# zhyever/PatchFusion

Measured on NVIDIA H100. Metric: tiles/s, higher is better.
Workload: dtype bf16

## Files before the change

patchfusion_b200/csrc/pf_attn.cu:

```cuda
#include <stdlib.h>

#include "pf_common.cuh"
#include "pf_kernels.h"

namespace pf {

constexpr int kQTile = 128, kKTile = 128, kHd = 64;
constexpr int kAttnWG = 2;
constexpr int kAttnThreads = kAttnWG * 128 + 32;
constexpr int kKVStages = 3;
constexpr int kTileBytes = 16384;
constexpr int kOffQ = 0;
constexpr int kOffKV = kTileBytes;
constexpr int kOffBar = kOffKV + kKVStages * 2 * kTileBytes;
constexpr int kAttnSmem = 1024 + kOffBar + 256;

struct AttnParams {
  CUtensorMap tmQK;
  CUtensorMap tmVt;
  int B, seq, heads, D;
  int n_qt;
  float scale_log2;
  __nv_bfloat16* out;
  int out_ld;
};

__device__ __forceinline__ float ex2_approx(float x) {
  float y;
  asm("ex2.approx.ftz.f32 %0, %1;" : "=f"(y) : "f"(x));
  return y;
}

__global__ void __launch_bounds__(kAttnThreads, 1) pf_attention_kernel(const __grid_constant__ AttnParams P) {
  extern __shared__ uint8_t smem_raw[];
  uint8_t* smem = reinterpret_cast<uint8_t*>((reinterpret_cast<uintptr_t>(smem_raw) + 1023) & ~uintptr_t(1023));
  uint64_t* bars = reinterpret_cast<uint64_t*>(smem + kOffBar);
  uint64_t* q_full = bars;
  uint64_t* kv_full = bars + 1;
  uint64_t* kv_empty = kv_full + kKVStages;
  const int warp = threadIdx.x >> 5, lane = threadIdx.x & 31;
  const int qt = blockIdx.x % P.n_qt;
  const int bh = blockIdx.x / P.n_qt;
  const int b = bh / P.heads, head = bh - b * P.heads;
  const int n_kv = (P.seq + kKTile - 1) / kKTile;
  constexpr int kProducer = kAttnWG * 4;

  if (warp == kProducer && lane == 0) {
    prefetch_tmap(&P.tmQK);
    prefetch_tmap(&P.tmVt);
    mbar_init(q_full, 1);
    for (int s = 0; s < kKVStages; ++s) { mbar_init(&kv_full[s], 1); mbar_init(&kv_empty[s], kAttnWG * 4); }
    fence_barrier_init();
  }
  __syncthreads();
  pdl_launch_dependents();
  pdl_wait();

  if (warp == kProducer) {
    if (elect_one()) {
      mbar_expect_tx(q_full, kTileBytes);
      tma_load_3d(smem + kOffQ, &P.tmQK, q_full, head * kHd, qt * kQTile, b);
      int st = 0; uint32_t ph = 0;
      for (int j = 0; j < n_kv; ++j) {
        mbar_wait(&kv_empty[st], ph ^ 1);
        uint8_t* sk = smem + kOffKV + st * 2 * kTileBytes;
        mbar_expect_tx(&kv_full[st], 2 * kTileBytes);
        tma_load_3d(sk, &P.tmQK, &kv_full[st], P.D + head * kHd, j * kKTile, b);
        const int vrow = (b * P.heads + head) * kHd;
        tma_load_2d(sk + kTileBytes, &P.tmVt, &kv_full[st], j * kKTile, vrow);
        tma_load_2d(sk + kTileBytes + 8192, &P.tmVt, &kv_full[st], j * kKTile + 64, vrow);
        if (++st == kKVStages) { st = 0; ph ^= 1; }
      }
    }
    return;
  }

  const int g = warp >> 2, wq = warp & 3;
  mbar_wait(q_full, 0);
  uint32_t qf[4][4];
  {
    const uint32_t base = smem_u32(smem + kOffQ);
    const int row = 64 * g + 16 * wq + (lane & 15);
#pragma unroll
    for (int k = 0; k < 4; ++k)
      ldmatrix_x4(base + row * 128 + ((((2 * k) + (lane >> 4)) ^ (row & 7)) << 4), qf[k]);
  }
  float o[32];
#pragma unroll
  for (int i = 0; i < 32; ++i) o[i] = 0.f;
  float m0 = -INFINITY, m1 = -INFINITY, l0 = 0.f, l1 = 0.f;
  const float sl2 = P.scale_log2;
  int st = 0; uint32_t ph = 0;
  for (int j = 0; j < n_kv; ++j) {
    mbar_wait(&kv_full[st], ph);
    const uint32_t sk = smem_u32(smem + kOffKV + st * 2 * kTileBytes);
    float s[64];
    wgmma_fence();
#pragma unroll
    for (int k = 0; k < 4; ++k) Wgmma<128>::rs(s, qf[k], wgmma_desc_k128(sk) + 2 * k, k);
    wgmma_commit();
    wgmma_wait<0>();
    const int kv_left = P.seq - j * kKTile;
    if (kv_left < kKTile) {
#pragma unroll
      for (int i = 0; i < 64; ++i) {
        const int key = 8 * (i >> 2) + 2 * (lane & 3) + (i & 1);
        if (key >= kv_left) s[i] = -INFINITY;
      }
    }
    float x0 = -INFINITY, x1 = -INFINITY;
#pragma unroll
    for (int i = 0; i < 64; i += 4) {
      x0 = fmaxf(x0, fmaxf(s[i], s[i + 1]));
      x1 = fmaxf(x1, fmaxf(s[i + 2], s[i + 3]));
    }
#pragma unroll
    for (int d = 1; d < 4; d <<= 1) {
      x0 = fmaxf(x0, __shfl_xor_sync(0xffffffffu, x0, d));
      x1 = fmaxf(x1, __shfl_xor_sync(0xffffffffu, x1, d));
    }
    const float n0 = fmaxf(m0, x0 * sl2), n1 = fmaxf(m1, x1 * sl2);
    const float c0 = ex2_approx(m0 - n0), c1 = ex2_approx(m1 - n1);
    m0 = n0; m1 = n1;
    float r0 = 0.f, r1 = 0.f;
#pragma unroll
    for (int i = 0; i < 64; i += 4) {
      s[i] = ex2_approx(fmaf(s[i], sl2, -n0));
      s[i + 1] = ex2_approx(fmaf(s[i + 1], sl2, -n0));
      s[i + 2] = ex2_approx(fmaf(s[i + 2], sl2, -n1));
      s[i + 3] = ex2_approx(fmaf(s[i + 3], sl2, -n1));
      r0 += s[i] + s[i + 1];
      r1 += s[i + 2] + s[i + 3];
    }
    l0 = l0 * c0 + r0;
    l1 = l1 * c1 + r1;
#pragma unroll
    for (int i = 0; i < 32; i += 4) {
      o[i] *= c0; o[i + 1] *= c0;
      o[i + 2] *= c1; o[i + 3] *= c1;
    }
    wgmma_fence();
#pragma unroll
    for (int kk = 0; kk < 8; ++kk) {
      const uint32_t pa[4] = {pack_bf16(s[8 * kk], s[8 * kk + 1]), pack_bf16(s[8 * kk + 2], s[8 * kk + 3]),
                              pack_bf16(s[8 * kk + 4], s[8 * kk + 5]), pack_bf16(s[8 * kk + 6], s[8 * kk + 7])};
      Wgmma<64>::rs(o, pa, wgmma_desc_k128(sk + kTileBytes + (kk >> 2) * 8192) + 2 * (kk & 3), 1);
    }
    wgmma_commit();
    wgmma_wait<0>();
    __syncwarp();
    if (lane == 0) mbar_arrive(&kv_empty[st]);
    if (++st == kKVStages) { st = 0; ph ^= 1; }
  }
#pragma unroll
  for (int d = 1; d < 4; d <<= 1) {
    l0 += __shfl_xor_sync(0xffffffffu, l0, d);
    l1 += __shfl_xor_sync(0xffffffffu, l1, d);
  }
  const float i0 = 1.f / l0, i1 = 1.f / l1;
  const int q0 = qt * kQTile + 64 * g + 16 * wq + (lane >> 2);
  __nv_bfloat16* ob = P.out + static_cast<size_t>(b) * P.seq * P.out_ld + head * kHd + 2 * (lane & 3);
#pragma unroll
  for (int jd = 0; jd < 8; ++jd) {
    if (q0 < P.seq)
      *reinterpret_cast<uint32_t*>(ob + static_cast<size_t>(q0) * P.out_ld + 8 * jd) = pack_bf16(o[4 * jd] * i0, o[4 * jd + 1] * i0);
    if (q0 + 8 < P.seq)
      *reinterpret_cast<uint32_t*>(ob + static_cast<size_t>(q0 + 8) * P.out_ld + 8 * jd) =
          pack_bf16(o[4 * jd + 2] * i1, o[4 * jd + 3] * i1);
  }
}

}

using namespace pf;

extern "C" int pf_attention(const void* qk, int32_t qk_ld, const void* vt, int32_t B, int32_t seq, int32_t seq_pad,
                            int32_t heads, float scale, void* out, int32_t out_ld, void* stream) {
  static bool attr_done[kMaxDevices] = {false};
  const int dev = current_device();
  if (!attr_done[dev]) {
    cudaError_t e = cudaFuncSetAttribute(pf_attention_kernel, cudaFuncAttributeMaxDynamicSharedMemorySize, kAttnSmem);
    if (e != cudaSuccess) return set_error("cudaFuncSetAttribute(pf_attention_kernel): %s", cudaGetErrorString(e));
    attr_done[dev] = true;
  }
  const int D = heads * kHd;
  if (B < 1 || seq < 1 || heads < 1) return set_error("pf_attention: empty problem");
  if (qk_ld % 8 || seq_pad % 8 || out_ld % 8) return set_error("pf_attention: strides must be multiples of 8");
  if (seq_pad < seq) return set_error("pf_attention: seq_pad %d < seq %d", seq_pad, seq);
  AttnParams P;
  if (tmap_3d_bf16(&P.tmQK, qk, 2 * D, seq, B, qk_ld, static_cast<uint64_t>(seq) * qk_ld, 64, 128, 1)) return 1;
  if (tmap_2d_bf16(&P.tmVt, vt, seq, static_cast<uint64_t>(B) * heads * kHd, seq_pad, 64, 64)) return 1;
  P.B = B; P.seq = seq; P.heads = heads; P.D = D;
  P.n_qt = (seq + kQTile - 1) / kQTile;
  P.scale_log2 = scale * 1.4426950408889634f;
  P.out = static_cast<__nv_bfloat16*>(out);
  P.out_ld = out_ld;
  note_work(4.0 * B * heads * static_cast<double>(seq) * seq * kHd, "attention B%d heads%d seq%d", B, heads, seq);
  cudaError_t le = launch_pdl(pf_attention_kernel, dim3(B * heads * P.n_qt), dim3(kAttnThreads), kAttnSmem,
                              static_cast<cudaStream_t>(stream), P);
  if (le != cudaSuccess) return set_error("pf_attention_kernel launch: %s", cudaGetErrorString(le));
  return check_launch("pf_attention_kernel");
}
```

patchfusion_b200/csrc/pf_common.cuh:

```cuda
#pragma once
#include <cuda.h>
#include <cuda_bf16.h>
#include <cuda_runtime.h>
#include <stdint.h>

namespace pf {

__device__ __forceinline__ uint32_t smem_u32(const void* p) {
  return static_cast<uint32_t>(__cvta_generic_to_shared(p));
}

__device__ __forceinline__ uint32_t lane_id() { return threadIdx.x & 31; }

__device__ __forceinline__ bool elect_one() {
  uint32_t pred = 0;
  asm volatile(
      "{\n\t"
      ".reg .pred P1;\n\t"
      "elect.sync _|P1, 0xffffffff;\n\t"
      "selp.b32 %0, 1, 0, P1;\n\t"
      "}\n"
      : "=r"(pred));
  return pred != 0;
}

__device__ __forceinline__ void mbar_init(uint64_t* bar, uint32_t count) {
  asm volatile("mbarrier.init.shared::cta.b64 [%0], %1;" ::"r"(smem_u32(bar)), "r"(count) : "memory");
}
__device__ __forceinline__ void fence_barrier_init() {
  asm volatile("fence.mbarrier_init.release.cluster;" ::: "memory");
}
__device__ __forceinline__ void mbar_expect_tx(uint64_t* bar, uint32_t bytes) {
  asm volatile("mbarrier.arrive.expect_tx.shared::cta.b64 _, [%0], %1;" ::"r"(smem_u32(bar)), "r"(bytes) : "memory");
}
__device__ __forceinline__ void mbar_arrive(uint64_t* bar) {
  asm volatile("mbarrier.arrive.shared::cta.b64 _, [%0];" ::"r"(smem_u32(bar)) : "memory");
}
__device__ __forceinline__ bool mbar_try_wait(uint64_t* bar, uint32_t parity) {
  uint32_t ok;
  asm volatile(
      "{\n\t"
      ".reg .pred P1;\n\t"
      "mbarrier.try_wait.parity.shared::cta.b64 P1, [%1], %2, %3;\n\t"
      "selp.b32 %0, 1, 0, P1;\n\t"
      "}\n"
      : "=r"(ok)
      : "r"(smem_u32(bar)), "r"(parity), "r"(20000u)
      : "memory");
  return ok != 0;
}
__device__ __forceinline__ bool mbar_test_wait(uint64_t* bar, uint32_t parity) {
  uint32_t ok;
  asm volatile(
      "{\n\t"
      ".reg .pred P1;\n\t"
      "mbarrier.test_wait.parity.shared::cta.b64 P1, [%1], %2;\n\t"
      "selp.b32 %0, 1, 0, P1;\n\t"
      "}\n"
      : "=r"(ok)
      : "r"(smem_u32(bar)), "r"(parity)
      : "memory");
  return ok != 0;
}
__device__ __forceinline__ void mbar_wait(uint64_t* bar, uint32_t parity) {
  uint32_t spins = 0;
  while (!mbar_try_wait(bar, parity)) {
    if (++spins > (1u << 20)) { __trap(); }
  }
}

__device__ __forceinline__ void pdl_launch_dependents() { asm volatile("griddepcontrol.launch_dependents;" ::: "memory"); }
__device__ __forceinline__ void pdl_wait() { asm volatile("griddepcontrol.wait;" ::: "memory"); }

__device__ __forceinline__ void fence_proxy_async_smem() { asm volatile("fence.proxy.async.shared::cta;" ::: "memory"); }

__device__ __forceinline__ void prefetch_tmap(const CUtensorMap* m) {
  asm volatile("prefetch.tensormap [%0];" ::"l"(reinterpret_cast<uint64_t>(m)) : "memory");
}
__device__ __forceinline__ void tma_load_2d(void* dst, const CUtensorMap* m, uint64_t* bar, int c0, int c1) {
  asm volatile(
      "cp.async.bulk.tensor.2d.shared::cluster.global.mbarrier::complete_tx::bytes [%0], [%1, {%3, %4}], [%2];"
      ::"r"(smem_u32(dst)), "l"(reinterpret_cast<uint64_t>(m)), "r"(smem_u32(bar)), "r"(c0), "r"(c1)
      : "memory");
}
__device__ __forceinline__ void tma_load_2d_mc(void* dst, const CUtensorMap* m, uint64_t* bar, int c0, int c1, uint16_t mask) {
  asm volatile(
      "cp.async.bulk.tensor.2d.shared::cluster.global.mbarrier::complete_tx::bytes.multicast::cluster [%0], [%1, {%3, %4}], [%2], %5;"
      ::"r"(smem_u32(dst)), "l"(reinterpret_cast<uint64_t>(m)), "r"(smem_u32(bar)), "r"(c0), "r"(c1), "h"(mask)
      : "memory");
}
__device__ __forceinline__ uint32_t cluster_ctarank() {
  uint32_t r;
  asm volatile("mov.u32 %0, %%cluster_ctarank;" : "=r"(r));
  return r;
}
__device__ __forceinline__ void cluster_sync_all() {
  asm volatile("barrier.cluster.arrive.release.aligned;\n\tbarrier.cluster.wait.acquire.aligned;" ::: "memory");
}
__device__ __forceinline__ void tma_load_3d(void* dst, const CUtensorMap* m, uint64_t* bar, int c0, int c1, int c2) {
  asm volatile(
      "cp.async.bulk.tensor.3d.shared::cluster.global.mbarrier::complete_tx::bytes [%0], [%1, {%3, %4, %5}], [%2];"
      ::"r"(smem_u32(dst)), "l"(reinterpret_cast<uint64_t>(m)), "r"(smem_u32(bar)), "r"(c0), "r"(c1), "r"(c2)
      : "memory");
}
__device__ __forceinline__ void tma_load_4d(void* dst, const CUtensorMap* m, uint64_t* bar, int c0, int c1, int c2,
                                            int c3) {
  asm volatile(
      "cp.async.bulk.tensor.4d.shared::cluster.global.mbarrier::complete_tx::bytes [%0], [%1, {%3, %4, %5, %6}], [%2];"
      ::"r"(smem_u32(dst)), "l"(reinterpret_cast<uint64_t>(m)), "r"(smem_u32(bar)), "r"(c0), "r"(c1), "r"(c2),
      "r"(c3)
      : "memory");
}

__device__ __forceinline__ void tma_store_2d(const CUtensorMap* m, const void* src, int c0, int c1) {
  asm volatile("cp.async.bulk.tensor.2d.global.shared::cta.bulk_group [%0, {%2, %3}], [%1];"
               ::"l"(reinterpret_cast<uint64_t>(m)), "r"(smem_u32(src)), "r"(c0), "r"(c1) : "memory");
}
__device__ __forceinline__ void tma_store_4d(const CUtensorMap* m, const void* src, int c0, int c1, int c2, int c3) {
  asm volatile("cp.async.bulk.tensor.4d.global.shared::cta.bulk_group [%0, {%2, %3, %4, %5}], [%1];"
               ::"l"(reinterpret_cast<uint64_t>(m)), "r"(smem_u32(src)), "r"(c0), "r"(c1), "r"(c2), "r"(c3) : "memory");
}
__device__ __forceinline__ void tma_reduce_add_2d(const CUtensorMap* m, const void* src, int c0, int c1) {
  asm volatile("cp.reduce.async.bulk.tensor.2d.global.shared::cta.add.tile.bulk_group [%0, {%2, %3}], [%1];"
               ::"l"(reinterpret_cast<uint64_t>(m)), "r"(smem_u32(src)), "r"(c0), "r"(c1) : "memory");
}
__device__ __forceinline__ void bulk_commit() { asm volatile("cp.async.bulk.commit_group;" ::: "memory"); }
__device__ __forceinline__ void bulk_wait_read0() { asm volatile("cp.async.bulk.wait_group.read 0;" ::: "memory"); }
__device__ __forceinline__ void bulk_wait_read1() { asm volatile("cp.async.bulk.wait_group.read 1;" ::: "memory"); }
__device__ __forceinline__ void bulk_wait0() { asm volatile("cp.async.bulk.wait_group 0;" ::: "memory"); }
__device__ __forceinline__ void st_shared_v2f(uint32_t addr, float a, float b) {
  asm volatile("st.shared.v2.f32 [%0], {%1, %2};" ::"r"(addr), "f"(a), "f"(b) : "memory");
}
__device__ __forceinline__ void st_shared_v4(uint32_t addr, uint32_t a, uint32_t b, uint32_t c, uint32_t d) {
  asm volatile("st.shared.v4.b32 [%0], {%1, %2, %3, %4};" ::"r"(addr), "r"(a), "r"(b), "r"(c), "r"(d) : "memory");
}
__device__ __forceinline__ void ld_shared_v4(uint32_t addr, uint32_t& a, uint32_t& b, uint32_t& c, uint32_t& d) {
  asm volatile("ld.shared.v4.b32 {%0, %1, %2, %3}, [%4];" : "=r"(a), "=r"(b), "=r"(c), "=r"(d) : "r"(addr) : "memory");
}
__device__ __forceinline__ void mbar_arrive_cluster(uint64_t* bar, uint32_t cta) {
  uint32_t remote;
  asm volatile("mapa.shared::cluster.u32 %0, %1, %2;" : "=r"(remote) : "r"(smem_u32(bar)), "r"(cta));
  asm volatile("mbarrier.arrive.shared::cluster.b64 _, [%0];" ::"r"(remote) : "memory");
}

__device__ __forceinline__ void ldmatrix_x4(uint32_t addr, uint32_t (&r)[4]) {
  asm volatile("ldmatrix.sync.aligned.m8n8.x4.shared.b16 {%0, %1, %2, %3}, [%4];"
               : "=r"(r[0]), "=r"(r[1]), "=r"(r[2]), "=r"(r[3]) : "r"(addr) : "memory");
}

__device__ __forceinline__ void stmatrix_x4(uint32_t addr, uint32_t r0, uint32_t r1, uint32_t r2, uint32_t r3) {
  asm volatile("stmatrix.sync.aligned.m8n8.x4.shared.b16 [%0], {%1, %2, %3, %4};"
               ::"r"(addr), "r"(r0), "r"(r1), "r"(r2), "r"(r3) : "memory");
}

__device__ __forceinline__ uint64_t wgmma_desc_k128(uint32_t saddr) {
// ... 247 lines not shown
```

patchfusion_b200/csrc/pf_gemm.cu:

```cuda
#include "pf_common.cuh"
#include "pf_kernels.h"

namespace pf {

constexpr int kBlockM = 128;
constexpr int kBlockK = 64;
constexpr int kATileBytes = kBlockM * kBlockK * 2;
constexpr int kEpiWarps = 8;
constexpr int kGemmThreads = (kEpiWarps + 1) * 32;
constexpr int kHaloThreads = (kEpiWarps + 3) * 32;
constexpr int kRsWarp0 = kEpiWarps;
constexpr int kMaxSmem = 227 * 1024;
constexpr int kXposeWarp = 16 * 32 * 4;
constexpr int kStageWarp = 2 * kXposeWarp;
constexpr int kBarBytes = 512;

__host__ __device__ constexpr int gemm_stage_bytes(int bn) { return kATileBytes + bn * kBlockK * 2; }
__host__ __device__ constexpr int gemm_stages(int bn) {
  return (kMaxSmem - 1024  - kBarBytes - kEpiWarps * kStageWarp) / gemm_stage_bytes(bn) < 8
             ? (kMaxSmem - 1024 - kBarBytes - kEpiWarps * kStageWarp) / gemm_stage_bytes(bn)
             : 8;
}

struct GemmKernelParams {
// ... 725 lines not shown
            int dy = d.taps == 9 ? tap / 3 - 1 : 0;
            int dx = d.taps == 9 ? tap % 3 - 1 : 0;
            for (int ch = 0; ch < d.chunks[s]; ++ch, ++kb) {
              const long long tl_w = tl.now();
              mbar_wait(&empty_bar[stage], phase ^ 1);
              tl.add(1, tl_w);
              uint8_t* sa = smem + stage * stage_bytes;
              uint8_t* sb = sa + kATileBytes;
              if (elect_one()) {
                mbar_expect_tx(&full_bar[stage], stage_bytes);
                if (d.a_mode == 0) tma_load_2d(sa, &P.tmA[s], &full_bar[stage], ch * kBlockK, c.m0);
                else tma_load_4d(sa, &P.tmA[s], &full_bar[stage], ch * kBlockK, c.x0 + dx, c.y0 + dy, c.img);
                if (MC) {
                  constexpr int half_rows = BN / 2;
                  tma_load_2d_mc(sb + it.rank * half_rows * 128, &P.tmBh, &full_bar[stage], kb * kBlockK,
                                 c.n0 + it.rank * half_rows, static_cast<uint16_t>(3));
                } else {
                  tma_load_2d(sb, &P.tmB, &full_bar[stage], kb * kBlockK, c.n0);
                }
              }
              if (++stage == stages) { stage = 0; phase ^= 1; }
            }
          }
        }
      }
      tl.add(2, tl_start);
      if (lane == 0) tl.flush(0, 3);
    }
  } else {
    EpiTma et;
    et.tm = &P.tmOut; et.stg_ptr = xpose + warp * kStageWarp; et.stg = smem_u32(et.stg_ptr); et.cur = 0;
    float* buf = reinterpret_cast<float*>(et.stg_ptr);
    const uint32_t a_off = static_cast<uint32_t>((warp >> 2) * 64 * 128);
    float acc[BN / 2];
    int stage = 0; uint32_t phase = 0;
    int rs = 0;
    GemmTimeline tl;
    const long long tl_start = tl.now();
    for (int ti = it.first; ti < it.count; ti += it.step) {
      const TileCoord c = decode_tile(d, it.tile(ti));
      tl.tile();
      const long long tl_main = tl.now();
      uint32_t accum = 0;
      for (int kb = 0; kb < P.k_steps; ++kb) {
        const long long tl_w = tl.now();
        mbar_wait(&full_bar[stage], phase);
        tl.add(1, tl_w);
        const uint32_t sa = smem_u32(smem + stage * stage_bytes);
        const uint64_t adesc = wgmma_desc_k128(sa + a_off);
        const uint64_t bdesc = wgmma_desc_k128(sa + kATileBytes);
        wgmma_fence();
#pragma unroll
        for (int k = 0; k < kBlockK / 16; ++k) Wgmma<BN>::ss(acc, adesc + 2 * k, bdesc + 2 * k, accum | k);
        wgmma_commit();
        accum = 1;
        wgmma_wait<1>();
        if (kb > 0) {
          release_stage<CL>(&empty_bar[rs], lane);
          if (++rs == stages) rs = 0;
        }
        if (++stage == stages) { stage = 0; phase ^= 1; }
      }
      wgmma_wait<0>();
      release_stage<CL>(&empty_bar[rs], lane);
      if (++rs == stages) rs = 0;
      tl.add(2, tl_main);
      const long long tl_epi = tl.now();
      epilogue_tile(d, c, acc, warp, lane, buf, &et);
      __syncwarp();
      tl.add(3, tl_epi);
    }
    if (lane == 0) bulk_wait0();
    tl.add(4, tl_start);
    if (lane == 0 && (warp & 3) == 0) tl.flush(3, 5);
  }
  __syncthreads();
  if (MC) cluster_sync_all();
}

constexpr int kPpStageBytes = kATileBytes + kPpBN * kBlockK * 2;
constexpr int kPpStages = (kMaxSmem - 1024  - kBarBytes - kEpiWarps * kStageWarp) / kPpStageBytes;
static_assert(kPpStages == 6, "pf_gemm_pp_kernel operand ring");
constexpr int kPpTurnBar = 1;

template <int ID>
__device__ __forceinline__ void named_bar_sync256() { asm volatile("bar.sync %0, 256;" ::"n"(ID) : "memory"); }
template <int ID>
__device__ __forceinline__ void named_bar_arrive256() { asm volatile("bar.arrive %0, 256;" ::"n"(ID) : "memory"); }

template <int S, int SC = 0>
__device__ __forceinline__ void epilogue_tile_vt(const GemmDesc& d, const float (&acc)[S], const TileCoord& c, int warp,
                                                 int lane) {
  const int q = lane & 3;
  int ro[2];
#pragma unroll
  for (int h = 0; h < 2; ++h) {
    const int m = c.m0 + 16 * warp + (lane >> 2) + 8 * h;
    const int b = m / d.vt_seq, tok = m - b * d.vt_seq;
    ro[h] = m < d.M ? b * d.vt_dim * d.vt_seq_pad + tok : -1;
  }
  for (int ch = 0; 32 * ch < 2 * S; ++ch) {
    const int lcol = c.n0 + ch * 32;
    if (lcol >= d.n_logical) break;
    float v[16];
    acc_chunk(ch, acc, v);
    if constexpr (SC != 0) epi_dequant(d, v, lcol + 2 * q, d.a_scale);
    epi_frag(d, v, lcol + 2 * q, false);
#pragma unroll
    for (int j = 0; j < 4; ++j) {
#pragma unroll
      for (int e = 0; e < 2; ++e) {
        const int n = lcol + 8 * j + 2 * q + e;
        if (n >= d.n_logical) continue;
        __nv_bfloat16* vp = d.vt + (n - d.vt_col0) * d.vt_seq_pad;
        if (ro[0] >= 0) vp[ro[0]] = __float2bfloat16(v[4 * j + e]);
        if (ro[1] >= 0) vp[ro[1]] = __float2bfloat16(v[4 * j + 2 + e]);
      }
    }
  }
}

template <bool F8, int S>
__device__ __forceinline__ void epilogue_tile_pp(const GemmDesc& d, EpiTma& et, const float (&acc)[S], const TileCoord& c,
                                                 int warp, int lane) {
  constexpr int SC = F8 ? 2 : 0;
  if (d.vt != nullptr && c.n0 >= d.vt_col0) epilogue_tile_vt<S, SC>(d, acc, c, warp, lane);
  else if (d.tma_out == 2) epilogue_tile_tma_f32<S, SC>(d, et, acc, c, warp, lane);
  else {
    if constexpr (F8) {
      if (d.out_e4m3) {
        epilogue_tile_tma_e4m3<S, true>(d, et, acc, c, warp, lane);
        return;
      }
    }
    epilogue_tile_tma_bf16<64, S, SC>(d, et, acc, c, warp, lane);
  }
}

template <bool MC, bool F8>
__device__ __forceinline__ void gemm_pp_body(const GemmKernelParams& P) {
  constexpr int CL = MC ? 2 : 1;
  constexpr int kKBlock = F8 ? 2 * kBlockK : kBlockK;
  extern __shared__ uint8_t smem_raw[];
  const GemmDesc& d = P.d;
  uint8_t* smem = reinterpret_cast<uint8_t*>((reinterpret_cast<uintptr_t>(smem_raw) + 1023) & ~uintptr_t(1023));
  uint8_t* stg = smem + kPpStages * kPpStageBytes;
  uint64_t* full_bar = reinterpret_cast<uint64_t*>(stg + kEpiWarps * kStageWarp);
  uint64_t* empty_bar = full_bar + kPpStages;

  const int warp = __shfl_sync(0xffffffffu, static_cast<int>(threadIdx.x >> 5), 0);
  const int lane = threadIdx.x & 31;
  pdl_launch_dependents();

  constexpr int kTmaWarp = kEpiWarps;
  if (warp == kTmaWarp && lane == 0) {
    prefetch_tmap(&P.tmA[0]);
    prefetch_tmap(MC ? &P.tmBh : &P.tmB);
    for (int s = 0; s < kPpStages; ++s) { mbar_init(&full_bar[s], 1); mbar_init(&empty_bar[s], 4 * CL); }
    prefetch_tmap(&P.tmOut);
    fence_barrier_init();
  }
  __syncthreads();
  if (MC) cluster_sync_all();
  const TileIter it = make_iter(d, P.total_tiles, CL);
  const int sub_log2 = d.block_n == 2 * kPpBN ? 1 : 0;
  const int items = it.first < it.count ? (it.count - 1 - it.first) / it.step + 1 : 0;
  const int tiles = items << sub_log2;
  pdl_wait();

  if (warp >= kEpiWarps) {
    if (warp == kTmaWarp) {
// ... 622 lines not shown
```

patchfusion_b200/engine.py:

```python
import ctypes as ct
import math

import torch
import torch.nn.functional as F

from . import lib, ops
from .ops import ACT_GELU, ACT_NONE, ACT_RELU, ACT_SOFTPLUS, call, pad_to, stream_ptr
from .params import FP8_LAYERS, VIT_FP8_LINEARS, WINDOW, branch_hparams, fusion_fp8_amax, fusion_precision, \
    guided_fusion_hparams, normed_attractors, vit_fp8_amax, vit_fp8_layers, vit_precision, DPT_FP8_CONVS, dpt_fp8_amax, \
    dpt_fp8_layers, dpt_precision, _get

BF16, F32 = torch.bfloat16, torch.float32


class Map:
    __slots__ = ('t', 'C')

    def __init__(self, t, C):
        self.t, self.C = t, C

    @property
    def B(self):
        return self.t.shape[0]

    @property
    def hw(self):
        return self.t.shape[1], self.t.shape[2]

    def rows(self):
        return self.t.view(-1, self.t.shape[-1])


class Engine:
    def __init__(self, config, state_dict, device, parts=('coarse', 'fine', 'fusion')):
        self.cfg = config
        self.parts = tuple(parts)
        self.dev = torch.device(device)
        self.P = tuple(_get(config, 'patch_process_shape'))
        branches = [b for b in ('coarse', 'fine') if b in self.parts or 'fusion' in self.parts]
        self.hp = {b: branch_hparams(_get(config, b + '_branch')) for b in branches}
        self.bcfg = {b: _get(config, b + '_branch') for b in branches}
        self.gf = guided_fusion_hparams(_get(config, 'guided_fusion'), self.P) if 'fusion' in self.parts else None
        self.bufs = {}
        self.arenas = {}
        self.generation = 0
        self._keep = []
        self.sd = {k: v.to(self.dev) for k, v in state_dict.items()}
        H, W = self.P
        assert H % 14 == 0 and W % 14 == 0
        self.gh, self.gw = H // 14, W // 14
        self.vit_fp8_static = vit_precision(config) == 'fp8_static'
        self.dpt_fp8_static = dpt_precision(config) == 'fp8_static'
        self.W = {}
        self._pack_all()
        self.sd = None
        self.c_branch = {b: self._c_branch(b) for b in ('coarse', 'fine') if b in self.parts}
        self.c_branch_bf16 = dict(self.c_branch)
        self.vit_amax = None
        self.dpt_amax = None
        self._branch_amax = {}
        if self.vit_fp8_static:
            self.set_vit_fp8_amax(vit_fp8_amax(config))
        if self.dpt_fp8_static:
            self.set_dpt_fp8_amax(dpt_fp8_amax(config))
        self.c_fusion = self._c_fusion() if 'fusion' in self.parts else None
        self.c_fusion_tiles = self.c_fusion
        self.fp8_static = 'fusion' in self.parts and fusion_precision(config) == 'fp8_static'
        self.fp8_amax = None
        self.calib = None
        if self.fp8_static:
            self.set_fp8_amax(fusion_fp8_amax(config))

    def buf(self, key, shape, dtype=BF16):
        k = (key, tuple(shape), dtype)
        t = self.bufs.get(k)
        if t is None:
            t = torch.zeros(shape, dtype=dtype, device=self.dev)
            self.bufs[k] = t
        return t

    def map(self, key, B, h, w, C):
        return Map(self.buf(key, (B, h, w, pad_to(C, 8))), C)

    def _w(self, k):
        return self.sd[k]

    def _dpt_conv(self, name, bias=True):
        return self._conv(name, bias=bias, fp8='keep_bf16' if self.dpt_fp8_static else None)

    def _conv(self, name, src_c=None, bias=True, fp8=None):
        b = self._w(name + '.bias') if bias and (name + '.bias') in self.sd else None
        if fp8:
            return ops.pack_weight_e4m3(self._w(name + '.weight'), b, src_c=src_c, keep_bf16=fp8 == 'keep_bf16')
        return ops.pack_weight(self._w(name + '.weight'), b, src_c=src_c)

    def _conv_bn(self, conv, bn, fp8=None):
        g, b = self._w(bn + '.weight'), self._w(bn + '.bias')
        m, v = self._w(bn + '.running_mean'), self._w(bn + '.running_var')
        scale = g / torch.sqrt(v + 1e-5)
        if fp8:
            return ops.pack_weight_e4m3(self._w(conv + '.weight'), None, scale=scale, shift=b - m * scale)
        return ops.pack_weight(self._w(conv + '.weight'), None, scale=scale, shift=b - m * scale)

    def _f32(self, k):
        return self._w(k).float().contiguous()

    def _pack_head(self, pre, C, hp, drop_rel):
        Wd = {}
        for n in ['seed_bin_regressor', 'seed_projector'] + ['projectors.%d' % i for i in range(4)] + \
                 ['attractors.%d' % i for i in range(4)]:
            Wd[n + '.0'] = self._conv(pre + n + '._net.0')
            w2, b2 = self._w(pre + n + '._net.2.weight'), self._w(pre + n + '._net.2.bias')
            if n.startswith('attractors') and normed_attractors(hp['bin_centers_type']):
                w2, b2 = w2[0::2].contiguous(), b2[0::2].contiguous()
            Wd[n + '.2'] = ops.pack_weight(w2, b2)
            if w2.shape[0] <= 16:
                Wd[n + '.tail'] = (w2.reshape(w2.shape[0], -1).float().contiguous(), b2.float().contiguous())
        w0 = self._w(pre + 'conditional_log_binomial.mlp.0.weight')
        b0 = self._w(pre + 'conditional_log_binomial.mlp.0.bias')
        E = hp['bin_embedding_dim']
        if drop_rel:
            w0 = torch.cat([w0[:, :32], w0[:, 33:]], 1).contiguous()
            Wd['clb.0'] = ops.pack_weight(w0, b0, src_c=[32, E])
        else:
            Wd['clb.0'] = ops.pack_weight(w0, b0, src_c=[32, 1, E])
        Wd['clb.tail'] = (self._w(pre + 'conditional_log_binomial.mlp.2.weight').reshape(4, -1).float().contiguous(),
                          self._f32(pre + 'conditional_log_binomial.mlp.2.bias'))
        return Wd

    def _pack_branch(self, which):
        pre = which + '_branch.'
        hp = self.hp[which]
        D, C, oc = hp['dim'], hp['features'], hp['out_channels']
        vit = pre + 'core.core.pretrained.'
        Wd = {}
        Wd['patch'] = ops.pack_weight(self._w(vit + 'patch_embed.proj.weight').reshape(D, 588),
                                      self._w(vit + 'patch_embed.proj.bias'))
        pe = self._w(vit + 'pos_embed').float()
        n = pe.shape[1] - 1
        s = int(math.sqrt(n))
        if (self.gh, self.gw) != (s, s):
            grid = pe[:, 1:].reshape(1, s, s, D).permute(0, 3, 1, 2)
            grid = F.interpolate(grid, scale_factor=((self.gh + 0.1) / s, (self.gw + 0.1) / s), mode='bicubic',
                                 antialias=False)
            assert grid.shape[-2:] == (self.gh, self.gw)
            pe = torch.cat([pe[:, :1], grid.permute(0, 2, 3, 1).reshape(1, self.gh * self.gw, D)], 1)
        Wd['pos'] = pe[0].contiguous()
        Wd['cls'] = self._f32(vit + 'cls_token').reshape(D)

        def lin(name):
            w, b = self._w(name + '.weight'), self._w(name + '.bias')
            if self.vit_fp8_static:
                return ops.pack_weight_e4m3(w, b, keep_bf16=True)
            return ops.pack_weight(w, b)
        for i in range(hp['depth']):
            p = vit + 'blocks.%d.' % i
            Wd['b%d' % i] = dict(
                n1w=self._f32(p + 'norm1.weight'), n1b=self._f32(p + 'norm1.bias'),
                n2w=self._f32(p + 'norm2.weight'), n2b=self._f32(p + 'norm2.bias'),
                qkv=lin(p + 'attn.qkv'), proj=ops.pack_weight(self._w(p + 'attn.proj.weight'), self._w(p + 'attn.proj.bias')),
# ... 159 lines not shown
        self.c_fusion = self._c_fusion({k: ct.addressof(arr) + 4 * i for i, k in enumerate(FP8_LAYERS)})
        self.fp8_amax = table

    def set_vit_fp8_amax(self, table):
        if table is None:
            self.vit_amax, self.c_branch = None, dict(self.c_branch_bf16)
            return
        self.vit_amax = dict(table)
        self._set_branch_amax(vit_fp8_layers(self.cfg), self.vit_amax, 'vit')

    def set_dpt_fp8_amax(self, table):
        self.dpt_amax = dict(table) if table is not None else None
        self._set_branch_amax(dpt_fp8_layers(self.cfg), self.dpt_amax, 'dpt')

    def _set_branch_amax(self, names, table, kind):
        if table is None:
            self._branch_amax.pop(kind, None)
        else:
            arr = (ct.c_float * len(names))(*[table[k] for k in names])
            self._keep.append(arr)
            self._branch_amax[kind] = {k: ct.addressof(arr) + 4 * i for i, k in enumerate(names)}

        def per_branch(kind, b):
            addr = self._branch_amax.get(kind)
            return None if addr is None else {k[len(b) + 1:]: a for k, a in addr.items() if k.startswith(b + '.')}
        self.c_branch = {b: self._c_branch(b, per_branch('vit', b), per_branch('dpt', b)) for b in self.c_branch_bf16}

    def _branch_struct(self, which):
        if self.calib is not None:
            return self.c_branch_bf16[which]
        if self.vit_fp8_static and self.vit_amax is None:
            raise RuntimeError("vit_precision 'fp8_static' needs the calibrated input scales `vit_fp8_amax`: run "
                               "PatchFusion.calibrate_fp8 (or tools/calibrate_fp8.py) first")
        if self.dpt_fp8_static and self.dpt_amax is None:
            raise RuntimeError("dpt_precision 'fp8_static' needs the calibrated input scales `dpt_fp8_amax`: run "
                               "PatchFusion.calibrate_fp8 (or tools/calibrate_fp8.py) first")
        return self.c_branch[which]

    def _fusion_struct(self):
        if self.calib is not None:
            return self.c_fusion_tiles
        if self.fp8_static and self.fp8_amax is None:
            raise RuntimeError("fusion_precision 'fp8_static' needs the calibrated input scales `fusion_fp8_amax`: run "
                               "PatchFusion.calibrate_fp8 (or tools/calibrate_fp8.py) first")
        return self.c_fusion

    def _c_fusion(self, amax=None):
        from . import stage
        Wf = self.W['fusion']
        F_ = stage.PfFusion()
        F_.H, F_.W = self.P
        for i in range(5):
            F_.fc[i] = stage.layer(Wf['fc%d' % i])
            F_.down[i][0], F_.down[i][1] = stage.layer(Wf['down%d.0' % i]), stage.layer(Wf['down%d.1' % i])
            F_.up[i][0], F_.up[i][1] = stage.layer(Wf['up%d.0' % (i + 1)]), stage.layer(Wf['up%d.1' % (i + 1)])
        F_.inc[0], F_.inc[1] = stage.layer(Wf['inc.0']), stage.layer(Wf['inc.1'])
        for i in range(6):
            F_.cv[i][0], F_.cv[i][1] = stage.layer(Wf['cv%d.0' % i]), stage.layer(Wf['cv%d.1' % i])
            L, g = Wf['g2l%d' % i], F_.g2l[i]
            g.C, g.heads, g.depth = L['C'], L['heads'], len(L['blocks'])
            g.ape, g.ape_rows = L['ape'].data_ptr(), L['ape'].shape[0]
            g.nw, g.nb, g.ones = L['nw'].data_ptr(), L['nb'].data_ptr(), L['ones'].data_ptr()
            blocks = (stage.PfG2LBlock * len(L['blocks']))()
            for b, bw in enumerate(L['blocks']):
                for k in ('n1w', 'n1b', 'n2w', 'n2b', 'table'):
                    setattr(blocks[b], k, bw[k].data_ptr())
                for k in ('qkv', 'proj', 'fc1', 'fc2'):
                    setattr(blocks[b], k, stage.layer(bw[k]))
            self._keep.append(blocks)
            g.blocks = blocks
        F_.head = self._c_head(Wf['head'], self.hp['coarse'], self.bcfg['coarse'], False, self.cfg)
        if amax is not None:
            for i in range(5):
                F_.down[i][0].a_amax, F_.down[i][1].a_amax = amax['down%d.0' % i], amax['down%d.1' % i]
                F_.up[i][0].a_amax, F_.up[i][1].a_amax = amax['up%d.0' % (i + 1)], amax['up%d.1' % (i + 1)]
            F_.inc[0].a_amax, F_.inc[1].a_amax = amax['inc.0'], amax['inc.1']
            for i in range(6):
                F_.cv[i][0].a_amax, F_.cv[i][1].a_amax = amax['cv%d.0' % i], amax['cv%d.1' % i]
        return F_

    def arena(self, name, nbytes):
        t = self.arenas.get(name)
        if t is None or t.numel() < nbytes:
            self.arenas[name] = t = torch.empty(int(nbytes) + 256, dtype=torch.uint8, device=self.dev)
            self.generation += 1
        return t

    @staticmethod
    def _view(arena, ptr, shape, dtype):
        off = ptr - arena.data_ptr()
        n = 1
        for s_ in shape:
            n *= s_
        nbytes = n * torch.empty((), dtype=dtype).element_size()
        assert 0 <= off and off + nbytes <= arena.numel()
        return arena[off:off + nbytes].view(dtype).view(shape)

    def _maps(self, arena, pf_maps):
        return [Map(self._view(arena, m.ptr, (m.B, m.H, m.W, m.ld), BF16), m.C) for m in pf_maps]

    def _tap_cb(self, arena, taps):
        def cb(user, name, ptr, is_f32, rows, cols, ld):
            if name.startswith(b'amaxv.') or name.startswith(b'amaxd.'):
                return
            t = self._view(arena, ptr, (rows, ld), (BF16, F32, torch.uint8)[is_f32])
            taps[name.decode()] = t[:, :cols].clone()
        return cb

    def _calib_cb(self, arena):
        def cb(user, name, ptr, is_f32, rows, cols, ld):
            name = name.decode()
            if not name.startswith('amax.'):
                return
            m = self._view(arena, ptr, (rows, ld), F32)[:, :cols].amax()
            k = name[5:]
            self.calib[k] = m if k not in self.calib else torch.maximum(self.calib[k], m)
        return cb

    def _calib_vit_cb(self, arena, which):
        prefixes = tuple(p for p, on in (('amaxv.', self.vit_fp8_static), ('amaxd.', self.dpt_fp8_static)) if on)

        def cb(user, name, ptr, is_f32, rows, cols, ld):
            name = name.decode()
            if not name.startswith(prefixes):
                return
            lo, hi = torch.aminmax(self._view(arena, ptr, (rows, ld), BF16)[:, :cols])
            m = torch.maximum(-lo, hi).float()
            k = '%s.%s' % (which, name[6:])
            self.calib[k] = m if k not in self.calib else torch.maximum(self.calib[k], m)
        return cb

    def branch(self, which, images, taps=None, ws=None):
        from . import stage
        cb = self._branch_struct(which)
        B = images.shape[0]
        need = stage.branch_workspace_bytes(cb, B)
        if ws is None:
            arena, off = self.arena(which, need), 0
        else:
            arena, off = ws
        assert images.dtype == F32 and images.is_contiguous() and off % 256 == 0 and off + need <= arena.numel()
        tap = self._tap_cb(arena, taps) if taps is not None else None
        if tap is None and self.calib is not None and (self.vit_fp8_static or self.dpt_fp8_static):
            tap = self._calib_vit_cb(arena, which)
        out = stage.branch_forward(cb, images, B, arena.data_ptr() + off, need, tap)
        H, W = self.P
        depth = self._view(arena, out.depth, (B, H, W), F32)
        feats = self._maps(arena, out.feats)
        if taps is not None:
            taps['rel'] = taps['rel'].view(B, H, W)
            for k_ in list(taps):
                if k_[0] == 'b' and k_[1:].isdigit():
                    m = feats[1 + int(k_[1:])]
                    taps[k_] = taps[k_].view(B, m.hw[0], m.hw[1], -1)
                elif k_ in ('seed', 'centers'):
                    m = feats[0 if k_ == 'seed' else 4]
                    taps[k_] = taps[k_].view(B, m.hw[0], m.hw[1], -1)
        return depth, feats

    def branch_bytes(self, which, B):
        from . import stage
        return stage.branch_workspace_bytes(self._branch_struct(which), B)

    @staticmethod
    def _pf_maps(maps):
        from . import stage
        arr = (stage.PfMap * len(maps))()
# ... 49 lines not shown
```

Baseline: 116.2.

## Pipeline attention QK and PV wgmmas with ping-pong warpgroup scheduling

Result: no change. 116.7 (median of 6 runs) (+0.5%).

```diff
diff --git a/patchfusion_b200/csrc/pf_attn.cu b/patchfusion_b200/csrc/pf_attn.cu
--- a/patchfusion_b200/csrc/pf_attn.cu
+++ b/patchfusion_b200/csrc/pf_attn.cu
@@ -9,6 +9,7 @@
 constexpr int kAttnWG = 2;
 constexpr int kAttnThreads = kAttnWG * 128 + 32;
 constexpr int kKVStages = 3;
+constexpr int kTurnBar = 1;
 constexpr int kTileBytes = 16384;
 constexpr int kOffQ = 0;
 constexpr int kOffKV = kTileBytes;
@@ -43,13 +44,14 @@
   const int bh = blockIdx.x / P.n_qt;
   const int b = bh / P.heads, head = bh - b * P.heads;
   const int n_kv = (P.seq + kKTile - 1) / kKTile;
+  const bool two_wg = P.seq - qt * kQTile > 64;
   constexpr int kProducer = kAttnWG * 4;
 
   if (warp == kProducer && lane == 0) {
     prefetch_tmap(&P.tmQK);
     prefetch_tmap(&P.tmVt);
     mbar_init(q_full, 1);
-    for (int s = 0; s < kKVStages; ++s) { mbar_init(&kv_full[s], 1); mbar_init(&kv_empty[s], kAttnWG * 4); }
+    for (int s = 0; s < kKVStages; ++s) { mbar_init(&kv_full[s], 1); mbar_init(&kv_empty[s], two_wg ? 8 : 4); }
     fence_barrier_init();
   }
   __syncthreads();
@@ -76,30 +78,41 @@
   }
 
   const int g = warp >> 2, wq = warp & 3;
+  if (g == 1 && !two_wg) return;
+  auto turn_wait = [&]() {
+    if (!two_wg) return;
+    if (g == 0) named_bar_sync256<kTurnBar>();
+    else named_bar_sync256<kTurnBar + 1>();
+  };
+  auto turn_pass = [&]() {
+    if (!two_wg) return;
+    if (g == 0) named_bar_arrive256<kTurnBar + 1>();
+    else named_bar_arrive256<kTurnBar>();
+  };
   mbar_wait(q_full, 0);
-  uint32_t qf[4][4];
-  {
-    const uint32_t base = smem_u32(smem + kOffQ);
-    const int row = 64 * g + 16 * wq + (lane & 15);
-#pragma unroll
-    for (int k = 0; k < 4; ++k)
-      ldmatrix_x4(base + row * 128 + ((((2 * k) + (lane >> 4)) ^ (row & 7)) << 4), qf[k]);
-  }
-  float o[32];
+  const uint64_t qdesc = wgmma_desc_k128(smem_u32(smem + kOffQ + g * 64 * 128));
+  const uint32_t kv0 = smem_u32(smem + kOffKV);
+  float s[64], o[32];
+  uint32_t p[32];
+  auto issue_qk = [&](uint32_t kv) {
+#pragma unroll
+    for (int k = 0; k < 4; ++k) Wgmma<128>::ss(s, qdesc + 2 * k, wgmma_desc_k128(kv) + 2 * k, k);
+    wgmma_commit();
+  };
+  auto issue_pv = [&](uint32_t kv) {
+#pragma unroll
+    for (int kk = 0; kk < 8; ++kk) {
+      const uint32_t pa[4] = {p[4 * kk], p[4 * kk + 1], p[4 * kk + 2], p[4 * kk + 3]};
+      Wgmma<64>::rs(o, pa, wgmma_desc_k128(kv + kTileBytes + (kk >> 2) * 8192) + 2 * (kk & 3), 1);
+    }
+    wgmma_commit();
+  };
 #pragma unroll
   for (int i = 0; i < 32; ++i) o[i] = 0.f;
   float m0 = -INFINITY, m1 = -INFINITY, l0 = 0.f, l1 = 0.f;
+  float c0, c1;
   const float sl2 = P.scale_log2;
-  int st = 0; uint32_t ph = 0;
-  for (int j = 0; j < n_kv; ++j) {
-    mbar_wait(&kv_full[st], ph);
-    const uint32_t sk = smem_u32(smem + kOffKV + st * 2 * kTileBytes);
-    float s[64];
-    wgmma_fence();
-#pragma unroll
-    for (int k = 0; k < 4; ++k) Wgmma<128>::rs(s, qf[k], wgmma_desc_k128(sk) + 2 * k, k);
-    wgmma_commit();
-    wgmma_wait<0>();
+  auto softmax = [&](int j) {
     const int kv_left = P.seq - j * kKTile;
     if (kv_left < kKTile) {
 #pragma unroll
@@ -120,7 +133,7 @@
       x1 = fmaxf(x1, __shfl_xor_sync(0xffffffffu, x1, d));
     }
     const float n0 = fmaxf(m0, x0 * sl2), n1 = fmaxf(m1, x1 * sl2);
-    const float c0 = ex2_approx(m0 - n0), c1 = ex2_approx(m1 - n1);
+    c0 = ex2_approx(m0 - n0); c1 = ex2_approx(m1 - n1);
     m0 = n0; m1 = n1;
     float r0 = 0.f, r1 = 0.f;
 #pragma unroll
@@ -134,24 +147,52 @@
     }
     l0 = l0 * c0 + r0;
     l1 = l1 * c1 + r1;
+  };
+  auto rescale_pack = [&]() {
 #pragma unroll
     for (int i = 0; i < 32; i += 4) {
       o[i] *= c0; o[i + 1] *= c0;
       o[i + 2] *= c1; o[i + 3] *= c1;
     }
-    wgmma_fence();
-#pragma unroll
-    for (int kk = 0; kk < 8; ++kk) {
-      const uint32_t pa[4] = {pack_bf16(s[8 * kk], s[8 * kk + 1]), pack_bf16(s[8 * kk + 2], s[8 * kk + 3]),
-                              pack_bf16(s[8 * kk + 4], s[8 * kk + 5]), pack_bf16(s[8 * kk + 6], s[8 * kk + 7])};
-      Wgmma<64>::rs(o, pa, wgmma_desc_k128(sk + kTileBytes + (kk >> 2) * 8192) + 2 * (kk & 3), 1);
-    }
-    wgmma_commit();
-    wgmma_wait<0>();
+#pragma unroll
+    for (int i = 0; i < 32; ++i) p[i] = pack_bf16(s[2 * i], s[2 * i + 1]);
+  };
+  auto release = [&](int st) {
     __syncwarp();
     if (lane == 0) mbar_arrive(&kv_empty[st]);
+  };
+
+  mbar_wait(&kv_full[0], 0);
+  if (g == 1) turn_wait();
+  wgmma_fence();
+  issue_qk(kv0);
+  turn_pass();
+  wgmma_wait<0>();
+  softmax(0);
+  rescale_pack();
+  int prev = 0, st = 1;
+  uint32_t ph = 0;
+  for (int j = 1; j < n_kv; ++j) {
+    mbar_wait(&kv_full[st], ph);
+    turn_wait();
+    wgmma_fence();
+    issue_qk(kv0 + st * 2 * kTileBytes);
+    issue_pv(kv0 + prev * 2 * kTileBytes);
+    turn_pass();
+    wgmma_wait<1>();
+    softmax(j);
+    wgmma_wait<0>();
+    release(prev);
+    rescale_pack();
+    prev = st;
     if (++st == kKVStages) { st = 0; ph ^= 1; }
   }
+  turn_wait();
+  wgmma_fence();
+  issue_pv(kv0 + prev * 2 * kTileBytes);
+  if (g == 0) turn_pass();
+  wgmma_wait<0>();
+  release(prev);
 #pragma unroll
   for (int d = 1; d < 4; d <<= 1) {
     l0 += __shfl_xor_sync(0xffffffffu, l0, d);
diff --git a/patchfusion_b200/csrc/pf_common.cuh b/patchfusion_b200/csrc/pf_common.cuh
--- a/patchfusion_b200/csrc/pf_common.cuh
+++ b/patchfusion_b200/csrc/pf_common.cuh
@@ -71,6 +71,11 @@
 
 __device__ __forceinline__ void pdl_launch_dependents() { asm volatile("griddepcontrol.launch_dependents;" ::: "memory"); }
 __device__ __forceinline__ void pdl_wait() { asm volatile("griddepcontrol.wait;" ::: "memory"); }
+
+template <int ID>
+__device__ __forceinline__ void named_bar_sync256() { asm volatile("bar.sync %0, 256;" ::"n"(ID) : "memory"); }
+template <int ID>
+__device__ __forceinline__ void named_bar_arrive256() { asm volatile("bar.arrive %0, 256;" ::"n"(ID) : "memory"); }
 
 __device__ __forceinline__ void fence_proxy_async_smem() { asm volatile("fence.proxy.async.shared::cta;" ::: "memory"); }
 
diff --git a/patchfusion_b200/csrc/pf_gemm.cu b/patchfusion_b200/csrc/pf_gemm.cu
--- a/patchfusion_b200/csrc/pf_gemm.cu
+++ b/patchfusion_b200/csrc/pf_gemm.cu
@@ -831,11 +831,6 @@
 constexpr int kPpStages = (kMaxSmem - 1024  - kBarBytes - kEpiWarps * kStageWarp) / kPpStageBytes;
 static_assert(kPpStages == 6, "pf_gemm_pp_kernel operand ring");
 constexpr int kPpTurnBar = 1;
-
-template <int ID>
-__device__ __forceinline__ void named_bar_sync256() { asm volatile("bar.sync %0, 256;" ::"n"(ID) : "memory"); }
-template <int ID>
-__device__ __forceinline__ void named_bar_arrive256() { asm volatile("bar.arrive %0, 256;" ::"n"(ID) : "memory"); }
 
 template <int S, int SC = 0>
 __device__ __forceinline__ void epilogue_tile_vt(const GemmDesc& d, const float (&acc)[S], const TileCoord& c, int warp,
diff --git a/patchfusion_b200/engine.py b/patchfusion_b200/engine.py
--- a/patchfusion_b200/engine.py
+++ b/patchfusion_b200/engine.py
@@ -1,4 +1,5 @@
 import ctypes as ct
+import gc
 import math
 
 import torch
@@ -29,6 +30,15 @@
 
     def rows(self):
         return self.t.view(-1, self.t.shape[-1])
+
+
+def _device_alloc(make):
+    try:
+        return make()
+    except torch.OutOfMemoryError:
+        gc.collect()
+        torch.cuda.empty_cache()
+        return make()
 
 
 class Engine:
@@ -75,7 +85,7 @@
         k = (key, tuple(shape), dtype)
         t = self.bufs.get(k)
         if t is None:
-            t = torch.zeros(shape, dtype=dtype, device=self.dev)
+            t = _device_alloc(lambda: torch.zeros(shape, dtype=dtype, device=self.dev))
             self.bufs[k] = t
         return t
 
@@ -401,7 +411,10 @@
     def arena(self, name, nbytes):
         t = self.arenas.get(name)
         if t is None or t.numel() < nbytes:
-            self.arenas[name] = t = torch.empty(int(nbytes) + 256, dtype=torch.uint8, device=self.dev)
+            self.arenas.pop(name, None)
+            t = None
+            self.arenas[name] = t = _device_alloc(
+                lambda: torch.empty(int(nbytes) + 256, dtype=torch.uint8, device=self.dev))
             self.generation += 1
         return t
 
```
